# kaegi/adaptive-sph

Hardware: AMD Instinct MI355X
Metric: particle-steps/sec (whole node), 2D dam-break N=1M DFSPH; 1/2/4/8 GPUs (higher is better)
Workload: dtype f32; 1 GPU; dam_break_1m: 2D dam-break, 1024x1024 = 1 048 576 uniform-h particles, HybridDFSPH; particles=1048576, solver=HybridDFSPH, parallelism=single GPU

## Files before the change

### adaptive_sph_amd/csrc/sph_api.hip

```cpp
#include <hip/hip_runtime.h>

#include <algorithm>
#include <chrono>
#include <cmath>
#include <cstdarg>
#include <cstdio>
#include <cstdlib>
#include <cstring>
#include <string>
#include <vector>

#include "sph_context.hpp"
#include "sph_lambda.hpp"

int Profiler::find(const char* name)
{
    for (size_t i = 0; i < recs.size(); i++)
        if (recs[i].name == name) return (int)i;
    recs.push_back(Rec{name, 0, 0, {}});
    return (int)recs.size() - 1;
}
bool Profiler::wants(const char* name) const
{
    return mode == 1 || mode == 3 || mode == 4 || (mode == 2 && (step_index & 7u) == 0u && strncmp(name, "density", 7) == 0);
// ... 181 lines not shown
        for (int k = 1; k < 4; k++) {
            r.min_x = fminf(r.min_x, s[k].min_x); r.min_y = fminf(r.min_y, s[k].min_y);
            r.max_x = fmaxf(r.max_x, s[k].max_x); r.max_y = fmaxf(r.max_y, s[k].max_y);
            r.h_max = fmaxf(r.h_max, s[k].h_max); r.h_min = fminf(r.h_min, s[k].h_min);
            r.min_cfl = fminf(r.min_cfl, s[k].min_cfl);
        }
        r.pad = seq - 1u;
        *out = r;
        if (seq) {
            __threadfence_system();
            ((volatile HeaderOut*)out)->pad = seq;
        }
    }
}

__global__ __launch_bounds__(1024) void k_header_ahead(const HeaderOut* __restrict__ partials, uint32_t nparts, const SolverCtrl* __restrict__ ctrl,
                                                       HeaderOut* __restrict__ out, const DeviceStatus* __restrict__ status, SolverCtrl* __restrict__ h_ctrl,
                                                       DeviceStatus* __restrict__ h_status, uint32_t seq)
{
    if (ctrl->done == 0u) {
        if (h_ctrl && threadIdx.x == 0) {
            SolverCtrl v = *ctrl;
            v.seq = seq - 1u;
            *h_ctrl = v;
            *h_status = *status;
            __threadfence_system();
            ((volatile SolverCtrl*)h_ctrl)->seq = seq;
        }
        return;
    }
    const float INF = __uint_as_float(0x7f800000u);
    HeaderOut o{INF, INF, -INF, -INF, 0.f, INF, INF, 0};
    for (uint32_t k0 = threadIdx.x; k0 < nparts; k0 += 4096u) {
        HeaderOut q[4];
#pragma unroll
        for (uint32_t u = 0; u < 4u; u++) q[u] = partials[min(k0 + 1024u * u, nparts - 1u)];
#pragma unroll
        for (uint32_t u = 0; u < 4u; u++) {
            o.min_x = fminf(o.min_x, q[u].min_x); o.min_y = fminf(o.min_y, q[u].min_y);
            o.max_x = fmaxf(o.max_x, q[u].max_x); o.max_y = fmaxf(o.max_y, q[u].max_y);
            o.h_max = fmaxf(o.h_max, q[u].h_max); o.h_min = fminf(o.h_min, q[u].h_min);
            o.min_cfl = fminf(o.min_cfl, q[u].min_cfl);
        }
    }
    o.min_x = wave_min(o.min_x); o.min_y = wave_min(o.min_y); o.max_x = wave_max(o.max_x); o.max_y = wave_max(o.max_y);
    o.h_max = wave_max(o.h_max); o.h_min = wave_min(o.h_min); o.min_cfl = wave_min(o.min_cfl);
    __shared__ HeaderOut s[16];
    const int lane = threadIdx.x & 63, w = threadIdx.x >> 6;
    if (lane == 0) s[w] = o;
    __syncthreads();
    if (threadIdx.x == 0) {
        HeaderOut r = s[0];
        for (int k = 1; k < 16; k++) {
            r.min_x = fminf(r.min_x, s[k].min_x); r.min_y = fminf(r.min_y, s[k].min_y);
            r.max_x = fmaxf(r.max_x, s[k].max_x); r.max_y = fmaxf(r.max_y, s[k].max_y);
            r.h_max = fmaxf(r.h_max, s[k].h_max); r.h_min = fminf(r.h_min, s[k].h_min);
            r.min_cfl = fminf(r.min_cfl, s[k].min_cfl);
        }
        *out = r;
        if (h_ctrl) {
            SolverCtrl v = *ctrl;
            v.seq = seq - 1u;
            *h_ctrl = v;
            *h_status = *status;
            __threadfence_system();
            ((volatile SolverCtrl*)h_ctrl)->seq = seq;
        }
    }
}

__global__ __launch_bounds__(256) void k_pack_upload(uint32_t n, const float* __restrict__ mass, const float2* __restrict__ pos,
                                                      const float2* __restrict__ velin, float4* __restrict__ pm, float2* __restrict__ vel,
                                                      uint32_t* __restrict__ orig, float* __restrict__ lvl, float* __restrict__ lvlold,
                                                      float* __restrict__ h2_next)
{
    uint32_t i = blockIdx.x * 256 + threadIdx.x;
    if (i >= n) return;
    float2 p = pos[i];
    pm[i] = make_float4(p.x, p.y, mass[i], 0.f);
    h2_next[i] = h_from_mass(mass[i], 1.f);
    vel[i] = velin[i];
    orig[i] = i;
    lvl[i] = __uint_as_float(0x7fc00000u);
// ... 330 lines not shown
}

extern "C" void sph_destroy(sph_ctx* c)
{
    if (!c) return;
    (void)hipSetDevice(c->device);
    if (c->stream) (void)hipStreamSynchronize(c->stream);
    if (c->stream2) (void)hipStreamSynchronize(c->stream2);
    dist_release(c);
    DevBuf* all[] = {&c->pm[0], &c->pm[1], &c->vel[0], &c->vel[1], &c->orig[0], &c->orig[1], &c->lvl[0], &c->lvl[1], &c->lvlold[0],
                     &c->lvlold[1], &c->vel_tmp, &c->key[0], &c->key[1], &c->val[0], &c->val[1], &c->sort_scratch, &c->cxy, &c->cell_start,
                     &c->cs_scratch, &c->hdr_ahead_partials, &c->h2n[0], &c->h2n[1], &c->lam_prev, &c->nl, &c->nlx, &c->tile_raw, &c->tile_h, &c->tile_h_ext, &c->lvl_changed_d, &c->lvl_tmp, &c->lvl_nrm, &c->lvl_state, &c->lvl_when, &c->lvl_mark, &c->lvl_queue, &c->nloff, &c->nlh, &c->flag_surface,
                     &c->flag_insufficient, &c->con_thr, &c->con_consumed, &c->con_h, &c->flag_reduced, &c->szc[0], &c->szc[1], &c->omega, &c->stash, &c->nl_ext, &c->nlx_ext, &c->nl_ok, &c->mrho, &c->pt0, &c->pt1, &c->prec0, &c->prec1, &c->xv, &c->rho, &c->lam_sum, &c->lam_grad, &c->wall_pl, &c->wall_cnt, &c->constf, &c->aii, &c->src, &c->p0, &c->p1, &c->pacc, &c->dens_err,
                     &c->stat, &c->ncount, &c->planes_d, &c->lam_lut, &c->dlam_lut, &c->hdr_partials, &c->hdr_out, &c->ctrl, &c->status,
                     &c->n_tiles, &c->red_partials, &c->scratch, &c->split_patterns, &c->akey[0], &c->akey[1], &c->aval[0], &c->aval[1], &c->acxy, &c->acell_start, &c->pm2,
                     &c->atile_raw, &c->atile_h, &c->inc_head, &c->inc_next, &c->inc_bsum, &c->inc_movers, &c->export_d_off, &c->export_d_idx,
                     &c->cand_rec, &c->cand_cls, &c->cand_cnt, &c->cand_off, &c->cand_idx, &c->cand_scan, &c->cand_red, &c->rnd_rec, &c->rnd_keys, &c->rnd_out, &c->rnd_max, &c->rnd_prev};
    for (auto b : all) b->release();
    if (c->hdr_host) (void)hipHostFree(c->hdr_host);
    if (c->ctrl_host) (void)hipHostFree(c->ctrl_host);
    if (c->status_host) (void)hipHostFree(c->status_host);
    if (c->lvl_changed) (void)hipHostFree(c->lvl_changed);
    for (auto& e : c->ev)
        if (e) (void)hipEventDestroy(e);
    if (c->ev_sync) (void)hipEventDestroy(c->ev_sync);
    if (c->stream) (void)hipStreamDestroy(c->stream);
    if (c->stream2) (void)hipStreamDestroy(c->stream2);
    if (c->ev_fork) (void)hipEventDestroy(c->ev_fork);
    delete c;
}

// ... 814 lines not shown
    int nb = (int)((n + 255) / 256);
    if (nb > HDR_BLOCKS) nb = HDR_BLOCKS;
    if (nb < 1) nb = 1;
    hipLaunchKernelGGL(k_header, dim3(nb), dim3(256), 0, s, c->pm[c->pcur].as<float4>(), c->vel[c->cur].as<float2>(), n, rest_density, from_mass,
                       c->h2n[c->cur].as<float>(), c->hdr_partials.as<HeaderOut>(), owned);
    c->publish_seq++;
    if (c->publish_seq == 0u) c->publish_seq = 1u;
    const bool mapped = out_dev == c->hdr_host_dev;
    hipLaunchKernelGGL(k_header_final, dim3(1), dim3(256), 0, s, c->hdr_partials.as<HeaderOut>(), nb, out_dev, mapped ? c->publish_seq : 0u);
    if (mapped) {
        c->hint_word = &((volatile HeaderOut*)c->hdr_host)->pad;
        c->hint_seq = c->publish_seq;
    }
}

void launch_header_ahead(sph_ctx* c, uint32_t nblocks, HeaderOut* out_dev, bool publish)
{
    ProfScope ps(&c->prof, "header_ahead", c->stream);
    uint32_t seq = 0;
    if (publish) {
        c->publish_seq++;
        if (c->publish_seq == 0u) c->publish_seq = 1u;
        seq = c->publish_seq;
        c->publish_folded = true;
    }
    hipLaunchKernelGGL(k_header_ahead, dim3(1), dim3(1024), 0, c->stream, c->hdr_ahead_partials.as<HeaderOut>(), nblocks, c->ctrl.as<SolverCtrl>(), out_dev,
                       c->status.as<DeviceStatus>(), publish ? c->ctrl_host_dev : (SolverCtrl*)nullptr, publish ? c->status_host_dev : (DeviceStatus*)nullptr, seq);
}

void launch_publish(sph_ctx* c)
{
    if (c->publish_folded) {
        c->publish_folded = false;
        return;
    }
    c->publish_seq++;
    if (c->publish_seq == 0u) c->publish_seq = 1u;
    hipLaunchKernelGGL(k_publish, dim3(1), dim3(64), 0, c->stream, c->ctrl.as<SolverCtrl>(), c->status.as<DeviceStatus>(), c->ctrl_host_dev,
                       c->status_host_dev, c->publish_seq);
}

void launch_check_neighborhood(sph_ctx* c, const SweepArgs& a)
// ... 5 lines not shown
```

### adaptive_sph_amd/csrc/sph_context.hpp

```cpp
#pragma once

#include <hip/hip_runtime.h>

#include <chrono>
#include <cstdarg>
#include <cstdio>
#include <string>
#include <vector>

#include "sph_internal.hpp"

struct DevBuf {
    void* p = nullptr;
    size_t bytes = 0;
    hipError_t ensure(size_t need)
    {
        if (need <= bytes) return hipSuccess;
        if (p) (void)hipFree(p);
        p = nullptr;
        bytes = 0;
        size_t grow = need + need / 4 + 256;
        hipError_t e = hipMalloc(&p, grow);
        if (e == hipSuccess) bytes = grow;
        return e;
// ... 141 lines not shown
        std::string shm_name;
        int rebalance_every = 0;
        DevBuf hist;
        uint32_t rebalances = 0;
        uint64_t stat_exchanges = 0, stat_bytes_sent = 0, stat_bytes_recv = 0, stat_allreduces = 0, stat_step0 = 0;
    } dist;

    GridP grid{};
    bool grid_valid = false;
    GridP fgrid{};
    int tile_ts = 0, tile_tsx = 0, tile_tsy = 0;
    DevBuf tile_raw, tile_h, tile_h_ext, nlx;
    DevBuf nloff, nlh;
    DevBuf akey[2], aval[2], acxy, acell_start, pm2;
    DevBuf atile_raw, atile_h;
    DevBuf inc_head, inc_next, inc_bsum, inc_movers;
    uint32_t inc_epoch = 0;
    int inc_radix_streak = 0;
    bool inc_count_valid = false;
    struct Ahead {
        bool valid = false;
        GridP g{};
        float h_max = 0.f, h_min = 0.f, rest_density = 0.f;
        int tile_ts = 0, tile_tsx = 0, tile_tsy = 0;
        uint64_t n = 0;
    } ahead;
    DevBuf hdr_ahead_partials;
    bool hdr_ahead = false;
    float hdr_ahead_rest_density = 0.f;
    DevBuf h2n[2];
    DevBuf lam_prev;
// ... 57 lines not shown
```

### adaptive_sph_amd/csrc/sph_internal.hpp

```cpp
#pragma once

#include <hip/hip_runtime.h>
#include <hip/hip_ext.h>
#include <stdint.h>

#include <string>
#include <vector>

#include "sph_device.h"
#include "sph_ffi.h"

struct Profiler {
    int mode = 0;
    uint64_t step_index = 0;
    struct Rec {
        std::string name;
        uint64_t launches = 0;
        double total_ms = 0;
        std::vector<float> samples;
    };
    struct Pending {
        int rec;
        hipEvent_t a, b;
        int slot;
// ... 47 lines not shown
    uint32_t done;
    uint32_t iters;
    uint32_t cur;
    uint32_t peer_error;
    uint32_t normal, singular, negative;
    float sum_err, max_err;
    uint32_t slot_done[2];
    uint32_t seq;
};

struct DeviceStatus {
    uint32_t error;
    uint32_t info;
};

struct CellKeyGen {
    const float4* pm;
    GridP g;
    const uint8_t* gone;
    uint32_t n_gone, gone_from;
    int clamp = 0;
};
int radix_sort_pairs(hipStream_t s, Profiler* prof, uint32_t* keyA, uint32_t* valA, uint32_t* keyB, uint32_t* valB,
                     uint32_t n, int bits, uint32_t* hist_scratch , const CellKeyGen* keygen = nullptr);
size_t radix_sort_scratch_elems(uint32_t n);
struct ReorderIO {
    const float4* pm_in;
    const float2* vel_in;
    const uint32_t* orig_in;
    const float *lvl_in, *lvlold_in;
    float4* pm_out;
    float2* vel_out;
    uint32_t* orig_out;
    float *lvl_out, *lvlold_out;
    uint32_t* cxy_out;
    const float* h2n_in;
    float* h2n_out;
    const float* lam_in;
    float* lam_prev_out;
    const uint8_t* szc_in;
    uint8_t* szc_out;
};
size_t incremental_sort_block_sums(uint32_t ncells);
void incremental_cell_sort_reorder(hipStream_t s, Profiler* prof, uint32_t n, const float4* pm_new, const IncClassifyP& q, bool classified,
                                   const uint32_t* cell_start_cur, uint32_t* key_out, uint32_t* cell_start_out, const ReorderIO& io, uint32_t* bsum, uint32_t* movers,
                                   uint32_t* movers_host);

void incremental_cell_sort_perm(hipStream_t s, Profiler* prof, uint32_t n, uint32_t n_prev, const CellKeyGen& kg, const IncClassifyP& q, const uint32_t* cell_start_cur,
                                uint32_t* key_out, uint32_t* perm_out, uint32_t* cell_start_out, uint32_t* bsum, uint32_t* movers, uint32_t* movers_host);

void launch_reorder(hipStream_t s, Profiler* prof, uint32_t n, GridP g, const uint32_t* sorted_key, const uint32_t* perm,
                    const float4* pm_in, const float2* vel_in, const uint32_t* orig_in, const float* lvl_in,
                    const float* lvlold_in, float4* pm_out, float2* vel_out, uint32_t* orig_out, float* lvl_out,
                    float* lvlold_out, uint32_t* cxy, const float* h2n_in = nullptr, float* h2n_out = nullptr,
                    const float* lam_in = nullptr, float* lam_prev_out = nullptr, void* cell_start_scratch = nullptr,
                    const uint8_t* szc_in = nullptr, uint8_t* szc_out = nullptr);
size_t cell_start_scratch_bytes();
void launch_cell_start(hipStream_t s, Profiler* prof, const uint32_t* sorted_key, uint32_t n, uint32_t ncells,
                       uint32_t* cell_start , void* scratch ,
                       bool count_zeroed = false );
void launch_tile_hmax(hipStream_t s, Profiler* prof, uint32_t n, const float4* pm, GridP g, int ts, int tsx, int tsy, uint32_t* raw,
// ... 123 lines not shown
    float* stash_first;
    int center_diff;
    int plain_propagate;
    const uint8_t* edge;
    int replay_step_lists;
    const float4* pm_cell;
};
void launch_max_disp(hipStream_t s, Profiler* prof, uint32_t n, const float4* pm_old, const float4* pm_new, uint32_t* out);
void launch_tile_redilate(hipStream_t s, Profiler* prof, int tsx, int tsy, int d, const uint32_t* raw, uint32_t* out);
void launch_level_detect(hipStream_t s, Profiler* prof, const SweepArgs& a, const LevelArgs& l);
void launch_level_propagate(hipStream_t s, Profiler* prof, const SweepArgs& a, const LevelArgs& l, uint32_t t, uint32_t* changed);
void launch_fill_stash(hipStream_t s, Profiler* prof, const SweepArgs& a, const LevelArgs& l, float* stash);
void launch_level_smooth(hipStream_t s, Profiler* prof, const SweepArgs& a, const LevelArgs& l, const float4* pm_new, const float* in, float* out);
void launch_classify(hipStream_t s, Profiler* prof, uint32_t n, const float4* pm, const float* level, uint8_t* size_class, const uint8_t* owned,
                     const uint32_t* orig, DeviceStatus* status, const sph_params* p);
void launch_header_ahead(sph_ctx* c, uint32_t nblocks, HeaderOut* out_dev, bool publish = false);
void launch_iisph2_scale(hipStream_t s, Profiler* prof, const SweepArgs& a);
void launch_check_aii(hipStream_t s, Profiler* prof, const SweepArgs& a);
void launch_vel_add_pacc(hipStream_t s, Profiler* prof, const SweepArgs& a);
void launch_integrate(hipStream_t s, Profiler* prof, const SweepArgs& a, float4* pm_out, int mode);

struct EditSrc {
    uint32_t obj;
    uint32_t set_idx;
};
struct EditSet {
    uint32_t fields;
    float mass, px, py, vx, vy, h2, h2_next, lvl, lvlold;
};
struct sph_ctx;
// ... 3 lines not shown
```

### adaptive_sph_amd/csrc/sph_sort.hip

```cpp
#include "sph_internal.hpp"

#define RS_ITEMS 32
#define RS_TILE (64 * RS_ITEMS)

template <int NB>
__device__ __forceinline__ uint64_t rs_peers(uint32_t d, bool valid)
{
    uint64_t peers = __ballot(valid);
#pragma unroll
    for (int b = 0; b < NB; b++) {
        const bool bit = (d >> b) & 1u;
        const uint64_t m = __ballot(bit);
        peers &= bit ? m : ~m;
    }
    return peers;
}

__device__ __forceinline__ uint32_t cell_key_of(const CellKeyGen& kg, uint32_t i)
{
    if (kg.gone && i < kg.n_gone && kg.gone[i] >= kg.gone_from) return kg.g.ncells;
    const float4 p = kg.pm[i];
    if (kg.clamp) return cell_key_clamped(kg.g, p.x, p.y);
    const int cx = (int)floorf(p.x / kg.g.cs) - kg.g.minx;
    const int cy = (int)floorf(p.y / kg.g.cs) - kg.g.miny;
// ... 294 lines not shown
    __syncthreads();
    uint32_t run = base_s + x - own;
    for (int k = 0; k < w; k++) run += ws[k];
#pragma unroll
    for (uint32_t u = 0; u < 4u; u++) {
        if (c0 + u < ncells) cell_start[c0 + u] = run;
        run += v[u];
        if (c0 + u + 1u == ncells) cell_start[ncells] = run;
    }
    if (blockIdx.x == 0 && tid == 0) {
        *movers_host = *movers;
        *movers = 0u;
    }
}

template <bool PERM>
__global__ __launch_bounds__(256) void k_inc_place_reorder(uint32_t n, IncGrid G, const uint32_t* __restrict__ cell_start_cur, const uint32_t* __restrict__ cell_start_nxt,
                                                            const uint32_t* __restrict__ nk, const uint8_t* __restrict__ mv, const uint32_t* __restrict__ next,
                                                            const unsigned long long* __restrict__ head, uint32_t epoch, const uint32_t* __restrict__ cxy_cur,
                                                            uint32_t* __restrict__ key_out, ReorderIO io, uint32_t* __restrict__ perm_out)
{
    const uint32_t i = blockIdx.x * 256 + threadIdx.x;
    if (i >= n) return;
    const uint32_t flag = mv[i];
    if (PERM && flag == 2u) return;
    const uint32_t c = nk[i];
    const bool mover = flag != 0u;
    const uint32_t own = mover ? 0u : cxy_cur[i];
    float4 pm;
    float2 vel;
    uint32_t orig = 0;
    float lvl = 0.f, lvlold = 0.f;
    if (!PERM) {
        pm = io.pm_in[i];
        vel = io.vel_in[i];
        orig = io.orig_in[i];
        lvl = io.lvl_in[i];
        lvlold = io.lvlold_in[i];
    }
    const unsigned long long h = head[c];
    const uint32_t first = cell_start_nxt[c];
    uint32_t b, e, r = 0;
    if (!mover) {
        const uint32_t k = (own & 0xffffu) + (own >> 16) * (uint32_t)G.cur.sx;
        b = cell_start_cur[k];
        e = i;
    } else {
        uint32_t eb;
        inc_cur_range(G, c, cell_start_cur, b, eb);
        e = i >= eb ? eb : b;
    }
    for (uint32_t j = b; j < e; j++) r += mv[j] ? 0u : 1u;
    if ((uint32_t)(h >> 32) == epoch)
        for (uint32_t m = (uint32_t)h; m; m = next[m - 1u]) r += (m - 1u < i) ? 1u : 0u;
    const uint32_t dst = first + r;
    key_out[dst] = c;
// ... 1 lines not shown
        perm_out[dst] = i;
        return;
    }
    io.pm_out[dst] = pm;
    io.vel_out[dst] = vel;
    io.orig_out[dst] = orig;
    io.lvl_out[dst] = lvl;
    io.lvlold_out[dst] = lvlold;
    if (io.h2n_in) io.h2n_out[dst] = io.h2n_in[i];
    if (io.lam_in) io.lam_prev_out[dst] = io.lam_in[i];
    if (io.szc_in) io.szc_out[dst] = io.szc_in[i];
    const uint32_t cy = c / (uint32_t)G.nxt.sx;
    io.cxy_out[dst] = (c - cy * (uint32_t)G.nxt.sx) | (cy << 16);
}

size_t incremental_sort_block_sums(uint32_t ncells) { return ((size_t)ncells + INC_CELLS - 1) / INC_CELLS; }

void incremental_cell_sort_reorder(hipStream_t s, Profiler* prof, uint32_t n, const float4* pm_new, const IncClassifyP& q, bool classified,
                                   const uint32_t* cell_start_cur, uint32_t* key_out, uint32_t* cell_start_out, const ReorderIO& io, uint32_t* bsum, uint32_t* movers,
                                   uint32_t* movers_host)
{
    const IncGrid G{q.cur, q.nxt};
    const uint32_t ncells = q.nxt.ncells, cblocks = (uint32_t)incremental_sort_block_sums(ncells);
    if (!classified) {
        ProfScope ps(prof, "inc_classify", s);
        hipLaunchKernelGGL(k_inc_classify, dim3((n + 255) / 256), dim3(256), 0, s, n, pm_new, q);
    }
    {
        ProfScope ps(prof, "inc_count", s);
        hipLaunchKernelGGL(k_inc_count, dim3(cblocks), dim3(INC_CELLS), 0, s, G, cell_start_cur, q.mv, q.next, q.head, q.epoch, cell_start_out, bsum, movers);
    }
    {
        ProfScope ps(prof, "inc_scan", s);
        hipLaunchKernelGGL(k_inc_scan, dim3(cblocks), dim3(256), 0, s, ncells, cell_start_out, bsum, movers, movers_host);
    }
    {
        ProfScope ps(prof, "inc_reorder", s);
        hipLaunchKernelGGL(k_inc_place_reorder<false>, dim3((n + 255) / 256), dim3(256), 0, s, n, G, cell_start_cur, cell_start_out, q.nk, q.mv, q.next, q.head,
                           q.epoch, q.cxy_cur, key_out, io, (uint32_t*)nullptr);
    }
}

void incremental_cell_sort_perm(hipStream_t s, Profiler* prof, uint32_t n, uint32_t n_prev, const CellKeyGen& kg, const IncClassifyP& q, const uint32_t* cell_start_cur,
                                uint32_t* key_out, uint32_t* perm_out, uint32_t* cell_start_out, uint32_t* bsum, uint32_t* movers, uint32_t* movers_host)
{
    const IncGrid G{q.cur, q.nxt};
    const uint32_t ncells = q.nxt.ncells, cblocks = (uint32_t)incremental_sort_block_sums(ncells);
    {
        ProfScope ps(prof, "inc_classify", s);
        hipLaunchKernelGGL(k_inc_classify_slab, dim3((n + 255) / 256), dim3(256), 0, s, n, n_prev, kg, q);
    }
    {
        ProfScope ps(prof, "inc_count", s);
        hipLaunchKernelGGL(k_inc_count, dim3(cblocks), dim3(INC_CELLS), 0, s, G, cell_start_cur, q.mv, q.next, q.head, q.epoch, cell_start_out, bsum, movers);
    }
    {
        ProfScope ps(prof, "inc_scan", s);
        hipLaunchKernelGGL(k_inc_scan, dim3(cblocks), dim3(256), 0, s, ncells, cell_start_out, bsum, movers, movers_host);
    }
    {
        ProfScope ps(prof, "inc_place", s);
        hipLaunchKernelGGL(k_inc_place_reorder<true>, dim3((n + 255) / 256), dim3(256), 0, s, n, G, cell_start_cur, cell_start_out, q.nk, q.mv, q.next, q.head, q.epoch,
                           q.cxy_cur, key_out, ReorderIO{}, perm_out);
    }
}

__global__ __launch_bounds__(256) void k_reorder(uint32_t n, GridP g, const uint32_t* __restrict__ sorted_key,
                                                  const uint32_t* __restrict__ perm, const float4* __restrict__ pm_in,
                                                  const float2* __restrict__ vel_in, const uint32_t* __restrict__ orig_in,
                                                  const float* __restrict__ lvl_in, const float* __restrict__ lvlold_in,
                                                  float4* __restrict__ pm_out, float2* __restrict__ vel_out,
                                                  uint32_t* __restrict__ orig_out, float* __restrict__ lvl_out,
                                                  float* __restrict__ lvlold_out, uint32_t* __restrict__ cxy,
                                                  const float* __restrict__ h2n_in, float* __restrict__ h2n_out,
                                                  const float* __restrict__ lam_in, float* __restrict__ lam_prev_out,
                                                  uint32_t* __restrict__ zero_word, const uint8_t* __restrict__ szc_in,
                                                  uint8_t* __restrict__ szc_out)
{
// ... 141 lines not shown
```

### adaptive_sph_amd/csrc/sph_step.hip

```cpp
#include <atomic>
#include <hip/hip_runtime.h>
#include <rccl/rccl.h>

#include <array>
#include <cmath>
#include <cstdlib>
#include <cstring>
#include <condition_variable>
#include <functional>
#include <memory>
#include <mutex>
#include <vector>

#include "sph_dist.hpp"

SweepArgs make_args(sph_ctx* c, const StepP& sp)
{
    SweepArgs a{};
    const int k = c->cur;
    a.g = c->fgrid;
    a.sp = sp;
    a.n = c->dist.on ? c->dist.n_tot : (uint32_t)c->n;
    a.exact = c->exact;
    a.cell_start = c->cell_start.as<uint32_t>();
// ... 268 lines not shown
static float* sel_pt0(Member& m) { return m.a.pt0; }
static float* sel_pt1(Member& m) { return m.a.pt1; }
static float* sel_rec0(Member& m) { return (float*)m.a.rec0; }
static float* sel_rec1(Member& m) { return (float*)m.a.rec1; }
static float* sel_lv_level(Member& m) { return m.lv_level; }
static float* sel_lv_when(Member& m) { return m.lv_when; }
static float* sel_lv_pmnew(Member& m) { return m.lv_pmnew; }

struct SolveQ {
    float max_avg_error;
    int residual_density;
    uint32_t max_iters;
    int tail;
    bool density_solver;
    int tot_slot = 0;
    uint32_t k = 1, upto = 2;
    void extend() { upto = k + std::max(1u, k / 4u); }
};
static int solve_sweep_a(Group& G, std::vector<Member>& M, const SolveQ& q, uint32_t k)
{
    const int multi = G.multi() ? 1 : 0;
    for (auto& m : M) {
        (void)hipSetDevice(m.c->device);
        if (m.n) launch_pressure_accel(m.c->stream, &m.c->prof, m.a, (int)k, q.residual_density, q.max_avg_error, q.max_iters, multi);
        else if (!multi) {
            SolverCtrl z{};
            z.done = 1u;
            z.slot_done[0] = z.slot_done[1] = 1u;
            z.cur = k & 1u;
            (void)hipMemcpyAsync(m.c->ctrl.p, &z, sizeof z, hipMemcpyHostToDevice, m.c->stream);
// ... 75 lines not shown
            if (m.n) launch_jacobi_update(m.c->stream, &m.c->prof, m.a, (int)k, q.residual_density, q.max_avg_error, q.max_iters, multi);
        }
        if ((rc = exchange_and_sweep_a(G, M, q, k + 1))) return rc;
    }
    for (auto& m : M) {
        (void)hipSetDevice(m.c->device);
        SolverCtrl* hand_host = handoff ? m.c->ctrl_host_dev + 1 : nullptr;
        uint32_t* gate_out = handoff ? (uint32_t*)(m.c->ctrl.as<SolverCtrl>() + 2) : nullptr;
        if (!m.n || q.tail == 0 ) {
            if (handoff) launch_solver_handoff(m.c->stream, &m.c->prof, m.c->ctrl.as<SolverCtrl>(), hand_host, gate_out);
            continue;
        }
        launch_solver_tail(m.c->stream, &m.c->prof, m.a, q.tail, m.c->pm[m.c->pcur ^ 1].as<float4>(), -1, q.residual_density,
                           q.max_avg_error, q.max_iters, hand_host, gate_out);
        if (q.tail == 1  && source_term_on_records(m.a)) m.a.xv_ok = true;
        if (q.tail >= 2  && m.a.hdr_partials) launch_header_ahead(m.c, (m.n + 255u) / 256u, m.c->hdr_host_dev, publish_next && !multi);
    }
    return SPH_OK;
}
static void solve_stats(Member& m, const SolveQ& q, const SolverCtrl& h)
{
    m.c->pressure_cur = h.cur;
    sph_solver_stats* st = q.density_solver ? &m.st.density_solver : &m.st.div_solver;
    st->iters = h.iters;
    st->converged = 1;
    st->normal_count = h.normal;
    st->singular_count = h.singular;
    st->negative_count = h.negative;
    st->avg_error = h.normal > 0 ? h.sum_err / (float)h.normal : NAN;
    st->max_error = h.max_err;
}
// ... 350 lines not shown
            std::swap(c->cell_start, c->acell_start);
            std::swap(c->pm[c->pcur ^ 1], c->pm2);
            c->cur = k ^ 1;
            c->pcur ^= 1;
            c->fgrid = ag;
            g = ag;
        } else if (n_sort) {
            const CellKeyGen kg{c->pm[c->pcur].as<float4>(), g, pre ? c->dist.cls.as<uint8_t>() : nullptr, pre ? c->dist.pre_cls_n : 0u, (uint32_t)SC_GONE_FROM};
            if (merge) {
                const size_t head_before = c->inc_head.bytes;
                HIPCHK(c, c->inc_head.ensure((size_t)g.ncells * 8));
                if (c->inc_head.bytes != head_before) HIPCHK(c, hipMemsetAsync(c->inc_head.p, 0, c->inc_head.bytes, s));
                HIPCHK(c, c->inc_next.ensure((size_t)c->cap * 4));
                HIPCHK(c, c->inc_bsum.ensure(incremental_sort_block_sums(g.ncells) * 4));
                if (!c->inc_movers.p) {
                    HIPCHK(c, c->inc_movers.ensure(4));
                    HIPCHK(c, hipMemsetAsync(c->inc_movers.p, 0, 4, s));
                }
                HIPCHK(c, c->acell_start.ensure(((size_t)g.ncells + 1) * sizeof(uint32_t)));
                if (++c->inc_epoch == 0u) c->inc_epoch = 1u;
                const IncClassifyP q{prev_grid, g, c->cxy.as<uint32_t>(), c->key[1].as<uint32_t>(), c->val[1].as<uint8_t>(), c->inc_next.as<uint32_t>(),
                                     c->inc_head.as<unsigned long long>(), c->inc_epoch};
                incremental_cell_sort_perm(s, prof, n_sort, n_prev, kg, q, c->cell_start.as<uint32_t>(), c->key[0].as<uint32_t>(), c->val[0].as<uint32_t>(),
                                           c->acell_start.as<uint32_t>(), c->inc_bsum.as<uint32_t>(), c->inc_movers.as<uint32_t>(),
                                           (uint32_t*)(c->ctrl_host_dev + 2) + 1);
                c->inc_count_valid = true;
                std::swap(c->cell_start, c->acell_start);
            } else {
                int res = radix_sort_pairs(s, prof, c->key[0].as<uint32_t>(), c->val[0].as<uint32_t>(), c->key[1].as<uint32_t>(),
                                           c->val[1].as<uint32_t>(), n_sort, ilog2_ceil(g.ncells + (pre ? 1u : 0u)), c->sort_scratch.as<uint32_t>(), &kg);
                if (res == 1) {
                    std::swap(c->key[0], c->key[1]);
// ... 534 lines not shown
        plan.on = true;
        plan.g = g;
        const uint32_t* movers_host = (const uint32_t*)(c->ctrl_host + 2) + 1;
        bool incremental = c->opt.inc_sort && c->grid_valid && c->fgrid.cs == cs && c->fgrid.ncells > 0 && g.ncells <= n + 4096u;
        if (incremental && c->inc_count_valid && *movers_host > n / (c->opt.inc_sort > 1 ? (uint32_t)c->opt.inc_sort : 3u)) {
            incremental = ++c->inc_radix_streak >= 8;
            if (incremental) c->inc_radix_streak = 0;
        }
        if (!incremental) return SPH_OK;
        hipStream_t s = c->stream;
        const size_t head_before = c->inc_head.bytes;
        HIPCHK(c, c->inc_head.ensure((size_t)g.ncells * 8));
        if (c->inc_head.bytes != head_before) HIPCHK(c, hipMemsetAsync(c->inc_head.p, 0, c->inc_head.bytes, s));
        HIPCHK(c, c->inc_next.ensure((size_t)c->cap * 4));
        HIPCHK(c, c->inc_bsum.ensure(incremental_sort_block_sums(g.ncells) * 4));
        if (!c->inc_movers.p) {
            HIPCHK(c, c->inc_movers.ensure(4));
            HIPCHK(c, hipMemsetAsync(c->inc_movers.p, 0, 4, s));
        }
        if (++c->inc_epoch == 0u) c->inc_epoch = 1u;
        plan.incremental = true;
        plan.q = IncClassifyP{c->fgrid, g, c->cxy.as<uint32_t>(), c->akey[1].as<uint32_t>(), c->aval[1].as<uint8_t>(), c->inc_next.as<uint32_t>(),
                              c->inc_head.as<unsigned long long>(), c->inc_epoch};
        M[0].a.inc = plan.q;
        return SPH_OK;
    };
    bool ahead_deferred = level_on;
    const std::function<int()> queue_ahead_build = [&]() -> int {
        sph_ctx* c = c0;
        if (ahead_deferred) return SPH_OK;
        c->ahead.valid = false;
        if (!plan.on) return SPH_OK;
        const uint32_t n = M[0].n;
        const GridP g = plan.g;
        hipStream_t s = c->stream;
        const int k = c->cur;
        const float4* integrated = c->pm[c->pcur ^ 1].as<float4>();
        if (plan.incremental) {
            const ReorderIO io{integrated, c->vel[k].as<float2>(), c->orig[k].as<uint32_t>(), c->lvl[k].as<float>(), c->lvlold[k].as<float>(), c->pm2.as<float4>(),
                               c->vel[k ^ 1].as<float2>(), c->orig[k ^ 1].as<uint32_t>(), c->lvl[k ^ 1].as<float>(), c->lvlold[k ^ 1].as<float>(), c->acxy.as<uint32_t>(),
                               c->h2n[k].as<float>(), c->h2n[k ^ 1].as<float>(),  nullptr, nullptr, c->szc[k].as<uint8_t>(), c->szc[k ^ 1].as<uint8_t>()};
            incremental_cell_sort_reorder(s, &c->prof, n, integrated, plan.q,  true, c->cell_start.as<uint32_t>(), c->akey[0].as<uint32_t>(),
                                          c->acell_start.as<uint32_t>(), io, c->inc_bsum.as<uint32_t>(), c->inc_movers.as<uint32_t>(),
                                          (uint32_t*)(c->ctrl_host_dev + 2) + 1);
            c->inc_count_valid = true;
        } else {
            const CellKeyGen kg{integrated, g, nullptr, 0u, (uint32_t)SC_GONE_FROM, 1};
            const int res = radix_sort_pairs(s, &c->prof, c->akey[0].as<uint32_t>(), c->aval[0].as<uint32_t>(), c->akey[1].as<uint32_t>(), c->aval[1].as<uint32_t>(), n,
                                             ilog2_ceil(g.ncells), c->sort_scratch.as<uint32_t>(), &kg);
            if (res == 1) {
                std::swap(c->akey[0], c->akey[1]);
                std::swap(c->aval[0], c->aval[1]);
            }
            launch_reorder(s, &c->prof, n, g, c->akey[0].as<uint32_t>(), c->aval[0].as<uint32_t>(), integrated, c->vel[k].as<float2>(), c->orig[k].as<uint32_t>(),
                           c->lvl[k].as<float>(), c->lvlold[k].as<float>(), c->pm2.as<float4>(), c->vel[k ^ 1].as<float2>(), c->orig[k ^ 1].as<uint32_t>(),
                           c->lvl[k ^ 1].as<float>(), c->lvlold[k ^ 1].as<float>(), c->acxy.as<uint32_t>(), c->h2n[k].as<float>(), c->h2n[k ^ 1].as<float>(),
                           c->lam_sum.as<float>(), c->lam_prev.as<float>(), c->cs_scratch.p, c->szc[k].as<uint8_t>(), c->szc[k ^ 1].as<uint8_t>());
            launch_cell_start(s, &c->prof, c->akey[0].as<uint32_t>(), n, g.ncells, c->acell_start.as<uint32_t>(), c->cs_scratch.p, true);
        }
// ... 58 lines not shown
        if (paced && (G.multi() || M[0].n > 0)) {
            const bool multi = G.multi();
            SolveQ qd{p->hybrid_dfsph_max_avg_divergence_error, 0, p->max_iters, T_VEL, false};
            SolveQ qs{p->hybrid_dfsph_max_avg_density_error, 1, p->max_iters, T_HYBRID, true};
            if ((rc = solve_paced(G, M, qd, pace_prediction(c0, M[0].n, c0->last_div_iters, c0->prev_div_iters)))) return rc;
            if ((rc = solve_queue(G, M, qd, true))) return rc;
            g_trace.mark(4);
            rec(3);
            if (multi && (rc = refresh_ghosts(G, M, sel_vel, 2, "vel"))) return rc;
            if (!p->hybrid_dfsph_non_pressure_accel_before_divergence_free)
                if ((rc = non_pressure())) return rc;
            rec(4);
            begin_solve(p->hybrid_dfsph_density_source_term == SPH_ONLY_DENSITY ? 2 : 1, 1);
            if ((rc = plan_ahead_build())) return rc;
            if ((rc = solve_paced(G, M, qs, pace_prediction(c0, M[0].n, c0->last_dens_iters, c0->prev_dens_iters)))) return rc;
            if ((rc = solve_queue(G, M, qs, false, true))) return rc;
            if ((rc = queue_ahead_build())) return rc;
            const bool final_solve = !level_on;
            if (multi && final_solve && (rc = G.comm->agree_guards_queued(G))) return rc;
            if ((rc = sync_ctrl(G, multi ? (final_solve ? SYNC_FINAL : SYNC_DEFER) : SYNC_AGREE))) return rc;
            for (auto& m : M) {
                solve_stats(m, qd, m.c->ctrl_host[1]);
                solve_stats(m, qs, *m.c->ctrl_host);
            }
            g_trace.mark(5);
            rec(5);
            break;
        }
        const bool chain_wanted = c0->opt.chain >= 0 ? c0->opt.chain == 1 : c0->last_div_iters == c0->prev_div_iters;
        const bool chain = (G.multi() || M[0].n > 0) && p->hybrid_dfsph_non_pressure_accel_before_divergence_free && chain_wanted;
// ... 306 lines not shown
```

Before: 2.434 billion particle-steps/s.

## Fuse incremental sort count and scan, fold header reduction into the kernel

Merges the separate incremental-sort count and scan kernels into a single kernel. Per-block local prefixes are finished with a last-block-done scan over block sums, and the block offset is added inside the place/reorder kernel, which also writes the final cell_start. The header-ahead reduction and host publish move into an extra block of that fused kernel, so the separate header_ahead launch after the density solve is skipped. This cuts kernel launches and a full pass over cell_start, at the cost of an extra scratch buffer, atomics-based grid completion detection, and the header now running later, after the build instead of right after the solver tail.

```diff
diff --git a/adaptive_sph_amd/csrc/sph_api.hip b/adaptive_sph_amd/csrc/sph_api.hip
--- a/adaptive_sph_amd/csrc/sph_api.hip
+++ b/adaptive_sph_amd/csrc/sph_api.hip
@@ -219,59 +219,9 @@
     }
 }
 
-__global__ __launch_bounds__(1024) void k_header_ahead(const HeaderOut* __restrict__ partials, uint32_t nparts, const SolverCtrl* __restrict__ ctrl,
-                                                       HeaderOut* __restrict__ out, const DeviceStatus* __restrict__ status, SolverCtrl* __restrict__ h_ctrl,
-                                                       DeviceStatus* __restrict__ h_status, uint32_t seq)
-{
-    if (ctrl->done == 0u) {
-        if (h_ctrl && threadIdx.x == 0) {
-            SolverCtrl v = *ctrl;
-            v.seq = seq - 1u;
-            *h_ctrl = v;
-            *h_status = *status;
-            __threadfence_system();
-            ((volatile SolverCtrl*)h_ctrl)->seq = seq;
-        }
-        return;
-    }
-    const float INF = __uint_as_float(0x7f800000u);
-    HeaderOut o{INF, INF, -INF, -INF, 0.f, INF, INF, 0};
-    for (uint32_t k0 = threadIdx.x; k0 < nparts; k0 += 4096u) {
-        HeaderOut q[4];
-#pragma unroll
-        for (uint32_t u = 0; u < 4u; u++) q[u] = partials[min(k0 + 1024u * u, nparts - 1u)];
-#pragma unroll
-        for (uint32_t u = 0; u < 4u; u++) {
-            o.min_x = fminf(o.min_x, q[u].min_x); o.min_y = fminf(o.min_y, q[u].min_y);
-            o.max_x = fmaxf(o.max_x, q[u].max_x); o.max_y = fmaxf(o.max_y, q[u].max_y);
-            o.h_max = fmaxf(o.h_max, q[u].h_max); o.h_min = fminf(o.h_min, q[u].h_min);
-            o.min_cfl = fminf(o.min_cfl, q[u].min_cfl);
-        }
-    }
-    o.min_x = wave_min(o.min_x); o.min_y = wave_min(o.min_y); o.max_x = wave_max(o.max_x); o.max_y = wave_max(o.max_y);
-    o.h_max = wave_max(o.h_max); o.h_min = wave_min(o.h_min); o.min_cfl = wave_min(o.min_cfl);
-    __shared__ HeaderOut s[16];
-    const int lane = threadIdx.x & 63, w = threadIdx.x >> 6;
-    if (lane == 0) s[w] = o;
-    __syncthreads();
-    if (threadIdx.x == 0) {
-        HeaderOut r = s[0];
-        for (int k = 1; k < 16; k++) {
-            r.min_x = fminf(r.min_x, s[k].min_x); r.min_y = fminf(r.min_y, s[k].min_y);
-            r.max_x = fmaxf(r.max_x, s[k].max_x); r.max_y = fmaxf(r.max_y, s[k].max_y);
-            r.h_max = fmaxf(r.h_max, s[k].h_max); r.h_min = fminf(r.h_min, s[k].h_min);
-            r.min_cfl = fminf(r.min_cfl, s[k].min_cfl);
-        }
-        *out = r;
-        if (h_ctrl) {
-            SolverCtrl v = *ctrl;
-            v.seq = seq - 1u;
-            *h_ctrl = v;
-            *h_status = *status;
-            __threadfence_system();
-            ((volatile SolverCtrl*)h_ctrl)->seq = seq;
-        }
-    }
+__global__ __launch_bounds__(1024) void k_header_ahead(HeaderAheadP a)
+{
+    header_ahead_block(a);
 }
 
 __global__ __launch_bounds__(256) void k_pack_upload(uint32_t n, const float* __restrict__ mass, const float2* __restrict__ pos,
@@ -632,7 +582,7 @@
                      &c->flag_insufficient, &c->con_thr, &c->con_consumed, &c->con_h, &c->flag_reduced, &c->szc[0], &c->szc[1], &c->omega, &c->stash, &c->nl_ext, &c->nlx_ext, &c->nl_ok, &c->mrho, &c->pt0, &c->pt1, &c->prec0, &c->prec1, &c->xv, &c->rho, &c->lam_sum, &c->lam_grad, &c->wall_pl, &c->wall_cnt, &c->constf, &c->aii, &c->src, &c->p0, &c->p1, &c->pacc, &c->dens_err,
                      &c->stat, &c->ncount, &c->planes_d, &c->lam_lut, &c->dlam_lut, &c->hdr_partials, &c->hdr_out, &c->ctrl, &c->status,
                      &c->n_tiles, &c->red_partials, &c->scratch, &c->split_patterns, &c->akey[0], &c->akey[1], &c->aval[0], &c->aval[1], &c->acxy, &c->acell_start, &c->pm2,
-                     &c->atile_raw, &c->atile_h, &c->inc_head, &c->inc_next, &c->inc_bsum, &c->inc_movers, &c->export_d_off, &c->export_d_idx,
+                     &c->atile_raw, &c->atile_h, &c->inc_head, &c->inc_next, &c->inc_bsum, &c->inc_movers, &c->inc_local, &c->export_d_off, &c->export_d_idx,
                      &c->cand_rec, &c->cand_cls, &c->cand_cnt, &c->cand_off, &c->cand_idx, &c->cand_scan, &c->cand_red, &c->rnd_rec, &c->rnd_keys, &c->rnd_out, &c->rnd_max, &c->rnd_prev};
     for (auto b : all) b->release();
     if (c->hdr_host) (void)hipHostFree(c->hdr_host);
@@ -1477,9 +1427,8 @@
     }
 }
 
-void launch_header_ahead(sph_ctx* c, uint32_t nblocks, HeaderOut* out_dev, bool publish)
-{
-    ProfScope ps(&c->prof, "header_ahead", c->stream);
+HeaderAheadP header_ahead_args(sph_ctx* c, uint32_t nblocks, HeaderOut* out_dev, bool publish)
+{
     uint32_t seq = 0;
     if (publish) {
         c->publish_seq++;
@@ -1487,8 +1436,14 @@
         seq = c->publish_seq;
         c->publish_folded = true;
     }
-    hipLaunchKernelGGL(k_header_ahead, dim3(1), dim3(1024), 0, c->stream, c->hdr_ahead_partials.as<HeaderOut>(), nblocks, c->ctrl.as<SolverCtrl>(), out_dev,
-                       c->status.as<DeviceStatus>(), publish ? c->ctrl_host_dev : (SolverCtrl*)nullptr, publish ? c->status_host_dev : (DeviceStatus*)nullptr, seq);
+    return HeaderAheadP{c->hdr_ahead_partials.as<HeaderOut>(), nblocks, c->ctrl.as<SolverCtrl>(), out_dev, c->status.as<DeviceStatus>(),
+                        publish ? c->ctrl_host_dev : (SolverCtrl*)nullptr, publish ? c->status_host_dev : (DeviceStatus*)nullptr, seq};
+}
+
+void launch_header_ahead(sph_ctx* c, uint32_t nblocks, HeaderOut* out_dev, bool publish)
+{
+    ProfScope ps(&c->prof, "header_ahead", c->stream);
+    hipLaunchKernelGGL(k_header_ahead, dim3(1), dim3(1024), 0, c->stream, header_ahead_args(c, nblocks, out_dev, publish));
 }
 
 void launch_publish(sph_ctx* c)
diff --git a/adaptive_sph_amd/csrc/sph_context.hpp b/adaptive_sph_amd/csrc/sph_context.hpp
--- a/adaptive_sph_amd/csrc/sph_context.hpp
+++ b/adaptive_sph_amd/csrc/sph_context.hpp
@@ -179,7 +179,7 @@
     DevBuf nloff, nlh;
     DevBuf akey[2], aval[2], acxy, acell_start, pm2;
     DevBuf atile_raw, atile_h;
-    DevBuf inc_head, inc_next, inc_bsum, inc_movers;
+    DevBuf inc_head, inc_next, inc_bsum, inc_movers, inc_local;
     uint32_t inc_epoch = 0;
     int inc_radix_streak = 0;
     bool inc_count_valid = false;
diff --git a/adaptive_sph_amd/csrc/sph_internal.hpp b/adaptive_sph_amd/csrc/sph_internal.hpp
--- a/adaptive_sph_amd/csrc/sph_internal.hpp
+++ b/adaptive_sph_amd/csrc/sph_internal.hpp
@@ -85,6 +85,69 @@
     uint32_t info;
 };
 
+struct HeaderAheadP {
+    const HeaderOut* partials;
+    uint32_t nparts;
+    const SolverCtrl* ctrl;
+    HeaderOut* out;
+    const DeviceStatus* status;
+    SolverCtrl* h_ctrl;
+    DeviceStatus* h_status;
+    uint32_t seq;
+};
+__device__ __forceinline__ void header_ahead_block(const HeaderAheadP& a)
+{
+    if (a.ctrl->done == 0u) {
+        if (a.h_ctrl && threadIdx.x == 0) {
+            SolverCtrl v = *a.ctrl;
+            v.seq = a.seq - 1u;
+            *a.h_ctrl = v;
+            *a.h_status = *a.status;
+            __threadfence_system();
+            ((volatile SolverCtrl*)a.h_ctrl)->seq = a.seq;
+        }
+        return;
+    }
+    const float INF = __uint_as_float(0x7f800000u);
+    HeaderOut o{INF, INF, -INF, -INF, 0.f, INF, INF, 0};
+    for (uint32_t k0 = threadIdx.x; k0 < a.nparts; k0 += 4096u) {
+        HeaderOut q[4];
+#pragma unroll
+        for (uint32_t u = 0; u < 4u; u++) q[u] = a.partials[min(k0 + 1024u * u, a.nparts - 1u)];
+#pragma unroll
+        for (uint32_t u = 0; u < 4u; u++) {
+            o.min_x = fminf(o.min_x, q[u].min_x); o.min_y = fminf(o.min_y, q[u].min_y);
+            o.max_x = fmaxf(o.max_x, q[u].max_x); o.max_y = fmaxf(o.max_y, q[u].max_y);
+            o.h_max = fmaxf(o.h_max, q[u].h_max); o.h_min = fminf(o.h_min, q[u].h_min);
+            o.min_cfl = fminf(o.min_cfl, q[u].min_cfl);
+        }
+    }
+    o.min_x = wave_min(o.min_x); o.min_y = wave_min(o.min_y); o.max_x = wave_max(o.max_x); o.max_y = wave_max(o.max_y);
+    o.h_max = wave_max(o.h_max); o.h_min = wave_min(o.h_min); o.min_cfl = wave_min(o.min_cfl);
+    __shared__ HeaderOut s[16];
+    const int lane = threadIdx.x & 63, w = threadIdx.x >> 6;
+    if (lane == 0) s[w] = o;
+    __syncthreads();
+    if (threadIdx.x == 0) {
+        HeaderOut r = s[0];
+        for (int k = 1; k < 16; k++) {
+            r.min_x = fminf(r.min_x, s[k].min_x); r.min_y = fminf(r.min_y, s[k].min_y);
+            r.max_x = fmaxf(r.max_x, s[k].max_x); r.max_y = fmaxf(r.max_y, s[k].max_y);
+            r.h_max = fmaxf(r.h_max, s[k].h_max); r.h_min = fminf(r.h_min, s[k].h_min);
+            r.min_cfl = fminf(r.min_cfl, s[k].min_cfl);
+        }
+        *a.out = r;
+        if (a.h_ctrl) {
+            SolverCtrl v = *a.ctrl;
+            v.seq = a.seq - 1u;
+            *a.h_ctrl = v;
+            *a.h_status = *a.status;
+            __threadfence_system();
+            ((volatile SolverCtrl*)a.h_ctrl)->seq = a.seq;
+        }
+    }
+}
+
 struct CellKeyGen {
     const float4* pm;
     GridP g;
@@ -114,8 +177,8 @@
 };
 size_t incremental_sort_block_sums(uint32_t ncells);
 void incremental_cell_sort_reorder(hipStream_t s, Profiler* prof, uint32_t n, const float4* pm_new, const IncClassifyP& q, bool classified,
-                                   const uint32_t* cell_start_cur, uint32_t* key_out, uint32_t* cell_start_out, const ReorderIO& io, uint32_t* bsum, uint32_t* movers,
-                                   uint32_t* movers_host);
+                                   const uint32_t* cell_start_cur, uint32_t* key_out, uint32_t* cell_start_out, const ReorderIO& io, uint32_t* local, uint32_t* bsum,
+                                   uint32_t* movers, uint32_t* movers_host, const HeaderAheadP* hdr = nullptr);
 
 void incremental_cell_sort_perm(hipStream_t s, Profiler* prof, uint32_t n, uint32_t n_prev, const CellKeyGen& kg, const IncClassifyP& q, const uint32_t* cell_start_cur,
                                 uint32_t* key_out, uint32_t* perm_out, uint32_t* cell_start_out, uint32_t* bsum, uint32_t* movers, uint32_t* movers_host);
@@ -269,6 +332,7 @@
 void launch_level_smooth(hipStream_t s, Profiler* prof, const SweepArgs& a, const LevelArgs& l, const float4* pm_new, const float* in, float* out);
 void launch_classify(hipStream_t s, Profiler* prof, uint32_t n, const float4* pm, const float* level, uint8_t* size_class, const uint8_t* owned,
                      const uint32_t* orig, DeviceStatus* status, const sph_params* p);
+HeaderAheadP header_ahead_args(sph_ctx* c, uint32_t nblocks, HeaderOut* out_dev, bool publish);
 void launch_header_ahead(sph_ctx* c, uint32_t nblocks, HeaderOut* out_dev, bool publish = false);
 void launch_iisph2_scale(hipStream_t s, Profiler* prof, const SweepArgs& a);
 void launch_check_aii(hipStream_t s, Profiler* prof, const SweepArgs& a);
diff --git a/adaptive_sph_amd/csrc/sph_sort.hip b/adaptive_sph_amd/csrc/sph_sort.hip
--- a/adaptive_sph_amd/csrc/sph_sort.hip
+++ b/adaptive_sph_amd/csrc/sph_sort.hip
@@ -332,13 +332,91 @@
     }
 }
 
-template <bool PERM>
+__global__ __launch_bounds__(INC_CELLS) void k_inc_count_scan(IncGrid G, const uint32_t* __restrict__ cell_start_cur, const uint8_t* __restrict__ mv,
+                                                               const uint32_t* __restrict__ next, const unsigned long long* __restrict__ head, uint32_t epoch,
+                                                               uint32_t* __restrict__ local, uint32_t* __restrict__ bsum, uint32_t* __restrict__ movers ,
+                                                               uint32_t* __restrict__ movers_host, uint32_t hdr, HeaderAheadP H)
+{
+    if (hdr && blockIdx.x == 0) {
+        header_ahead_block(H);
+        return;
+    }
+    __shared__ uint32_t ws[INC_CELLS / 64], wm[INC_CELLS / 64], last_s;
+    const uint32_t blk = blockIdx.x - hdr, nblk = gridDim.x - hdr;
+    const uint32_t tid = threadIdx.x, lane = tid & 63u, w = tid >> 6;
+    const uint32_t c = blk * (uint32_t)INC_CELLS + tid;
+    uint32_t cnt = 0, listed = 0;
+    if (c < G.nxt.ncells) {
+        uint32_t b, e;
+        inc_cur_range(G, c, cell_start_cur, b, e);
+        const unsigned long long h = head[c];
+        for (uint32_t j = b; j < e; j++) cnt += mv[j] ? 0u : 1u;
+        if ((uint32_t)(h >> 32) == epoch)
+            for (uint32_t m = (uint32_t)h; m; m = next[m - 1u]) listed++;
+        cnt += listed;
+    }
+    uint32_t x = cnt, y = listed;
+#pragma unroll
+    for (int o = 1; o < 64; o <<= 1) {
+        const uint32_t u = __shfl_up(x, o, 64);
+        if ((int)lane >= o) x += u;
+    }
+    for (int o = 32; o > 0; o >>= 1) y += (uint32_t)__shfl_xor((int)y, o, 64);
+    if (lane == 63u) ws[w] = x;
+    if (lane == 0u) wm[w] = y;
+    __syncthreads();
+    uint32_t run = x - cnt;
+    for (uint32_t k = 0; k < w; k++) run += ws[k];
+    if (c < G.nxt.ncells) local[c] = run;
+    if (tid == 0u) {
+        uint32_t t = 0, m = 0;
+        for (int k = 0; k < INC_CELLS / 64; k++) {
+            t += ws[k];
+            m += wm[k];
+        }
+        bsum[blk] = t;
+        if (m) atomicAdd(movers, m);
+        __threadfence();
+        last_s = atomicAdd(movers + 1, 1u) == nblk - 1u ? 1u : 0u;
+    }
+    __syncthreads();
+    if (!last_s) return;
+    __threadfence();
+    uint32_t carry = 0;
+    for (uint32_t base = 0; base < nblk; base += (uint32_t)INC_CELLS) {
+        const uint32_t k = base + tid;
+        const uint32_t v = k < nblk ? ((const volatile uint32_t*)bsum)[k] : 0u;
+        x = v;
+#pragma unroll
+        for (int o = 1; o < 64; o <<= 1) {
+            const uint32_t u = __shfl_up(x, o, 64);
+            if ((int)lane >= o) x += u;
+        }
+        __syncthreads();
+        if (lane == 63u) ws[w] = x;
+        __syncthreads();
+        run = carry + x - v;
+        for (uint32_t j = 0; j < w; j++) run += ws[j];
+        if (k < nblk) bsum[k] = run;
+        for (int j = 0; j < INC_CELLS / 64; j++) carry += ws[j];
+    }
+    if (tid == 0u) {
+        bsum[nblk] = carry;
+        *movers_host = atomicExch(movers, 0u);
+        atomicExch(movers + 1, 0u);
+    }
+}
+
+template <bool PERM, bool LOCAL>
 __global__ __launch_bounds__(256) void k_inc_place_reorder(uint32_t n, IncGrid G, const uint32_t* __restrict__ cell_start_cur, const uint32_t* __restrict__ cell_start_nxt,
                                                             const uint32_t* __restrict__ nk, const uint8_t* __restrict__ mv, const uint32_t* __restrict__ next,
                                                             const unsigned long long* __restrict__ head, uint32_t epoch, const uint32_t* __restrict__ cxy_cur,
-                                                            uint32_t* __restrict__ key_out, ReorderIO io, uint32_t* __restrict__ perm_out)
+                                                            uint32_t* __restrict__ key_out, ReorderIO io, uint32_t* __restrict__ perm_out,
+                                                            const uint32_t* __restrict__ bpre, uint32_t* __restrict__ cell_start_fin)
 {
     const uint32_t i = blockIdx.x * 256 + threadIdx.x;
+    if (LOCAL && i <= G.nxt.ncells)
+        cell_start_fin[i] = i < G.nxt.ncells ? cell_start_nxt[i] + bpre[i / (uint32_t)INC_CELLS] : bpre[(G.nxt.ncells + (uint32_t)INC_CELLS - 1u) / (uint32_t)INC_CELLS];
     if (i >= n) return;
     const uint32_t flag = mv[i];
     if (PERM && flag == 2u) return;
@@ -357,7 +435,7 @@
         lvlold = io.lvlold_in[i];
     }
     const unsigned long long h = head[c];
-    const uint32_t first = cell_start_nxt[c];
+    const uint32_t first = cell_start_nxt[c] + (LOCAL ? bpre[c / (uint32_t)INC_CELLS] : 0u);
     uint32_t b, e, r = 0;
     if (!mover) {
         const uint32_t k = (own & 0xffffu) + (own >> 16) * (uint32_t)G.cur.sx;
@@ -389,19 +467,41 @@
     io.cxy_out[dst] = (c - cy * (uint32_t)G.nxt.sx) | (cy << 16);
 }
 
-size_t incremental_sort_block_sums(uint32_t ncells) { return ((size_t)ncells + INC_CELLS - 1) / INC_CELLS; }
+size_t incremental_sort_block_sums(uint32_t ncells) { return ((size_t)ncells + INC_CELLS - 1) / INC_CELLS + 1; }
 
 void incremental_cell_sort_reorder(hipStream_t s, Profiler* prof, uint32_t n, const float4* pm_new, const IncClassifyP& q, bool classified,
-                                   const uint32_t* cell_start_cur, uint32_t* key_out, uint32_t* cell_start_out, const ReorderIO& io, uint32_t* bsum, uint32_t* movers,
-                                   uint32_t* movers_host)
+                                   const uint32_t* cell_start_cur, uint32_t* key_out, uint32_t* cell_start_out, const ReorderIO& io, uint32_t* local, uint32_t* bsum,
+                                   uint32_t* movers, uint32_t* movers_host, const HeaderAheadP* hdr)
 {
     const IncGrid G{q.cur, q.nxt};
-    const uint32_t ncells = q.nxt.ncells, cblocks = (uint32_t)incremental_sort_block_sums(ncells);
+    const uint32_t ncells = q.nxt.ncells, cblocks = (ncells + INC_CELLS - 1) / INC_CELLS;
     if (!classified) {
         ProfScope ps(prof, "inc_classify", s);
         hipLaunchKernelGGL(k_inc_classify, dim3((n + 255) / 256), dim3(256), 0, s, n, pm_new, q);
     }
     {
+        ProfScope ps(prof, "inc_count_scan", s);
+        hipLaunchKernelGGL(k_inc_count_scan, dim3(cblocks + (hdr ? 1u : 0u)), dim3(INC_CELLS), 0, s, G, cell_start_cur, q.mv, q.next, q.head, q.epoch, local, bsum, movers,
+                           movers_host, hdr ? 1u : 0u, hdr ? *hdr : HeaderAheadP{});
+    }
+    {
+        ProfScope ps(prof, "inc_reorder", s);
+        const uint32_t threads = n > ncells + 1u ? n : ncells + 1u;
+        hipLaunchKernelGGL((k_inc_place_reorder<false, true>), dim3((threads + 255) / 256), dim3(256), 0, s, n, G, cell_start_cur, local, q.nk, q.mv, q.next, q.head,
+                           q.epoch, q.cxy_cur, key_out, io, (uint32_t*)nullptr, bsum, cell_start_out);
+    }
+}
+
+void incremental_cell_sort_perm(hipStream_t s, Profiler* prof, uint32_t n, uint32_t n_prev, const CellKeyGen& kg, const IncClassifyP& q, const uint32_t* cell_start_cur,
+                                uint32_t* key_out, uint32_t* perm_out, uint32_t* cell_start_out, uint32_t* bsum, uint32_t* movers, uint32_t* movers_host)
+{
+    const IncGrid G{q.cur, q.nxt};
+    const uint32_t ncells = q.nxt.ncells, cblocks = (ncells + INC_CELLS - 1) / INC_CELLS;
+    {
+        ProfScope ps(prof, "inc_classify", s);
+        hipLaunchKernelGGL(k_inc_classify_slab, dim3((n + 255) / 256), dim3(256), 0, s, n, n_prev, kg, q);
+    }
+    {
         ProfScope ps(prof, "inc_count", s);
         hipLaunchKernelGGL(k_inc_count, dim3(cblocks), dim3(INC_CELLS), 0, s, G, cell_start_cur, q.mv, q.next, q.head, q.epoch, cell_start_out, bsum, movers);
     }
@@ -410,33 +510,9 @@
         hipLaunchKernelGGL(k_inc_scan, dim3(cblocks), dim3(256), 0, s, ncells, cell_start_out, bsum, movers, movers_host);
     }
     {
-        ProfScope ps(prof, "inc_reorder", s);
-        hipLaunchKernelGGL(k_inc_place_reorder<false>, dim3((n + 255) / 256), dim3(256), 0, s, n, G, cell_start_cur, cell_start_out, q.nk, q.mv, q.next, q.head,
-                           q.epoch, q.cxy_cur, key_out, io, (uint32_t*)nullptr);
-    }
-}
-
-void incremental_cell_sort_perm(hipStream_t s, Profiler* prof, uint32_t n, uint32_t n_prev, const CellKeyGen& kg, const IncClassifyP& q, const uint32_t* cell_start_cur,
-                                uint32_t* key_out, uint32_t* perm_out, uint32_t* cell_start_out, uint32_t* bsum, uint32_t* movers, uint32_t* movers_host)
-{
-    const IncGrid G{q.cur, q.nxt};
-    const uint32_t ncells = q.nxt.ncells, cblocks = (uint32_t)incremental_sort_block_sums(ncells);
-    {
-        ProfScope ps(prof, "inc_classify", s);
-        hipLaunchKernelGGL(k_inc_classify_slab, dim3((n + 255) / 256), dim3(256), 0, s, n, n_prev, kg, q);
-    }
-    {
-        ProfScope ps(prof, "inc_count", s);
-        hipLaunchKernelGGL(k_inc_count, dim3(cblocks), dim3(INC_CELLS), 0, s, G, cell_start_cur, q.mv, q.next, q.head, q.epoch, cell_start_out, bsum, movers);
-    }
-    {
-        ProfScope ps(prof, "inc_scan", s);
-        hipLaunchKernelGGL(k_inc_scan, dim3(cblocks), dim3(256), 0, s, ncells, cell_start_out, bsum, movers, movers_host);
-    }
-    {
         ProfScope ps(prof, "inc_place", s);
-        hipLaunchKernelGGL(k_inc_place_reorder<true>, dim3((n + 255) / 256), dim3(256), 0, s, n, G, cell_start_cur, cell_start_out, q.nk, q.mv, q.next, q.head, q.epoch,
-                           q.cxy_cur, key_out, ReorderIO{}, perm_out);
+        hipLaunchKernelGGL((k_inc_place_reorder<true, false>), dim3((n + 255) / 256), dim3(256), 0, s, n, G, cell_start_cur, cell_start_out, q.nk, q.mv, q.next, q.head, q.epoch,
+                           q.cxy_cur, key_out, ReorderIO{}, perm_out, (const uint32_t*)nullptr, (uint32_t*)nullptr);
     }
 }
 
diff --git a/adaptive_sph_amd/csrc/sph_step.hip b/adaptive_sph_amd/csrc/sph_step.hip
--- a/adaptive_sph_amd/csrc/sph_step.hip
+++ b/adaptive_sph_amd/csrc/sph_step.hip
@@ -306,6 +306,7 @@
     int tail;
     bool density_solver;
     int tot_slot = 0;
+    bool header_in_build = false;
     uint32_t k = 1, upto = 2;
     void extend() { upto = k + std::max(1u, k / 4u); }
 };
@@ -411,7 +412,7 @@
         launch_solver_tail(m.c->stream, &m.c->prof, m.a, q.tail, m.c->pm[m.c->pcur ^ 1].as<float4>(), -1, q.residual_density,
                            q.max_avg_error, q.max_iters, hand_host, gate_out);
         if (q.tail == 1  && source_term_on_records(m.a)) m.a.xv_ok = true;
-        if (q.tail >= 2  && m.a.hdr_partials) launch_header_ahead(m.c, (m.n + 255u) / 256u, m.c->hdr_host_dev, publish_next && !multi);
+        if (q.tail >= 2  && m.a.hdr_partials && !q.header_in_build) launch_header_ahead(m.c, (m.n + 255u) / 256u, m.c->hdr_host_dev, publish_next && !multi);
     }
     return SPH_OK;
 }
@@ -792,8 +793,8 @@
                 HIPCHK(c, c->inc_next.ensure((size_t)c->cap * 4));
                 HIPCHK(c, c->inc_bsum.ensure(incremental_sort_block_sums(g.ncells) * 4));
                 if (!c->inc_movers.p) {
-                    HIPCHK(c, c->inc_movers.ensure(4));
-                    HIPCHK(c, hipMemsetAsync(c->inc_movers.p, 0, 4, s));
+                    HIPCHK(c, c->inc_movers.ensure(8));
+                    HIPCHK(c, hipMemsetAsync(c->inc_movers.p, 0, 8, s));
                 }
                 HIPCHK(c, c->acell_start.ensure(((size_t)g.ncells + 1) * sizeof(uint32_t)));
                 if (++c->inc_epoch == 0u) c->inc_epoch = 1u;
@@ -1358,9 +1359,10 @@
         if (c->inc_head.bytes != head_before) HIPCHK(c, hipMemsetAsync(c->inc_head.p, 0, c->inc_head.bytes, s));
         HIPCHK(c, c->inc_next.ensure((size_t)c->cap * 4));
         HIPCHK(c, c->inc_bsum.ensure(incremental_sort_block_sums(g.ncells) * 4));
+        HIPCHK(c, c->inc_local.ensure((size_t)g.ncells * 4));
         if (!c->inc_movers.p) {
-            HIPCHK(c, c->inc_movers.ensure(4));
-            HIPCHK(c, hipMemsetAsync(c->inc_movers.p, 0, 4, s));
+            HIPCHK(c, c->inc_movers.ensure(8));
+            HIPCHK(c, hipMemsetAsync(c->inc_movers.p, 0, 8, s));
         }
         if (++c->inc_epoch == 0u) c->inc_epoch = 1u;
         plan.incremental = true;
@@ -1370,6 +1372,7 @@
         return SPH_OK;
     };
     bool ahead_deferred = level_on;
+    bool header_in_build = false, header_publish = false;
     const std::function<int()> queue_ahead_build = [&]() -> int {
         sph_ctx* c = c0;
         if (ahead_deferred) return SPH_OK;
@@ -1384,9 +1387,12 @@
             const ReorderIO io{integrated, c->vel[k].as<float2>(), c->orig[k].as<uint32_t>(), c->lvl[k].as<float>(), c->lvlold[k].as<float>(), c->pm2.as<float4>(),
                                c->vel[k ^ 1].as<float2>(), c->orig[k ^ 1].as<uint32_t>(), c->lvl[k ^ 1].as<float>(), c->lvlold[k ^ 1].as<float>(), c->acxy.as<uint32_t>(),
                                c->h2n[k].as<float>(), c->h2n[k ^ 1].as<float>(),  nullptr, nullptr, c->szc[k].as<uint8_t>(), c->szc[k ^ 1].as<uint8_t>()};
+            HeaderAheadP hdr{};
+            if (header_in_build) hdr = header_ahead_args(c, (n + 255u) / 256u, c->hdr_host_dev, header_publish);
             incremental_cell_sort_reorder(s, &c->prof, n, integrated, plan.q,  true, c->cell_start.as<uint32_t>(), c->akey[0].as<uint32_t>(),
-                                          c->acell_start.as<uint32_t>(), io, c->inc_bsum.as<uint32_t>(), c->inc_movers.as<uint32_t>(),
-                                          (uint32_t*)(c->ctrl_host_dev + 2) + 1);
+                                          c->acell_start.as<uint32_t>(), io, c->inc_local.as<uint32_t>(), c->inc_bsum.as<uint32_t>(), c->inc_movers.as<uint32_t>(),
+                                          (uint32_t*)(c->ctrl_host_dev + 2) + 1, header_in_build ? &hdr : nullptr);
+            header_in_build = false;
             c->inc_count_valid = true;
         } else {
             const CellKeyGen kg{integrated, g, nullptr, 0u, (uint32_t)SC_GONE_FROM, 1};
@@ -1475,6 +1481,8 @@
             begin_solve(p->hybrid_dfsph_density_source_term == SPH_ONLY_DENSITY ? 2 : 1, 1);
             if ((rc = plan_ahead_build())) return rc;
             if ((rc = solve_paced(G, M, qs, pace_prediction(c0, M[0].n, c0->last_dens_iters, c0->prev_dens_iters)))) return rc;
+            qs.header_in_build = header_in_build = plan.on && plan.incremental && !ahead_deferred && M[0].a.hdr_partials != nullptr;
+            header_publish = true;
             if ((rc = solve_queue(G, M, qs, false, true))) return rc;
             if ((rc = queue_ahead_build())) return rc;
             const bool final_solve = !level_on;
```

Measured after the change: 2.415 billion particle-steps/s. No clear change (-0.8%).
